# dmlc/difacto

Hardware: AMD Instinct MI355X
Metric: examples/sec (FM SGD worker step, Criteo-shape, V_dim=64) (higher is better)
Workload: dtype f32

## Files before the change

difacto_amd/csrc/dfh_localize.hip:

```cpp
#ifndef DFH_LOCALIZE_HIP_
#define DFH_LOCALIZE_HIP_
#include "dfh_internal.h"

namespace dfh {

constexpr int LOC_OVERSAMPLE = 8;
constexpr int LOC_MAX_BUCKETS = 1024;
constexpr int LOC_BIG_BUCKETS = 4096;
constexpr int LOC_AVG_BUCKET = 384;
constexpr int LOC_MIN_AVG = 48;
constexpr int LOC_MAX_AVG = 700;
constexpr int LOC_LDS_CAP = 1024;
#ifndef DFH_LOC_TILE
#define DFH_LOC_TILE 2048
#endif
#ifndef DFH_LOC_TILE_THREADS
#define DFH_LOC_TILE_THREADS 1024
#endif
constexpr int LOC_TILE = DFH_LOC_TILE;
constexpr int LOC_TILE_THREADS = DFH_LOC_TILE_THREADS;
constexpr int LOC_PER_THREAD = LOC_TILE / LOC_TILE_THREADS;
constexpr int LOC_SORT_THREADS = 256;
constexpr int LOC_EMIT_THREADS = 256;

struct LocView {
  const uint64_t* raw;
  uint32_t n;
  uint64_t max_index;
  int P;
  int bstride;
  int ntiles;
  int force_global;
  int tb;
  uint32_t nrows;
  const uint32_t* offset;
  const uint32_t* rowid;
  uint64_t* smp_key;
  uint32_t* smp_pos;
  uint32_t* smp_rank;
  uint64_t* spl_key;
  uint32_t* spl_pos;
  uint32_t* packed;
  uint32_t* run_off;
  uint32_t* btotal;
  uint32_t* bstart;
  uint64_t* bkeys;
  uint32_t* bpos;
  uint64_t* skeys;
  uint32_t* spos;
  uint64_t* first_key;
  uint64_t* last_key;
  uint32_t* nheads;
  uint32_t* lh;
  uint32_t* split_n;
};

struct SegListsOut {
  uint2* mid;
  SegEnt* mid_ent;
  uint2* hot;
  SegEnt* hot_ent;
  uint2* few;
  SegEnt* few_ent;
};

__device__ __forceinline__ uint64_t make_key(uint64_t id, uint64_t max_index) {
  const uint64_t m = (max_index == ~0ULL) ? (id == ~0ULL ? 0ULL : id) : id % max_index;
  return reverse_bytes(m);
}

constexpr int LOC_XCDS = 8;

__device__ __forceinline__ bool comp_less(uint64_t ka, uint32_t pa, uint64_t kb, uint32_t pb) {
  return ka < kb || (ka == kb && pa < pb);
}

template <bool MAX>
__device__ __forceinline__ uint32_t wave_inclusive(uint32_t x) {
#define DFH_DPP_STEP(ctrl, row_mask)                                                                      \
  {                                                                                                       \
    const uint32_t y = (uint32_t)__builtin_amdgcn_update_dpp(0, (int)x, ctrl, row_mask, 0xf, false);    \
    x = MAX ? max(x, y) : x + y;                                                                          \
  }
  DFH_DPP_STEP(0x111, 0xf)
  DFH_DPP_STEP(0x112, 0xf)
  DFH_DPP_STEP(0x114, 0xf)
  DFH_DPP_STEP(0x118, 0xf)
  DFH_DPP_STEP(0x142, 0xa)
  DFH_DPP_STEP(0x143, 0xc)
#undef DFH_DPP_STEP
  return x;
}

template <bool MAX, int NWAVES>
__device__ __forceinline__ uint32_t block_exclusive(uint32_t val, uint32_t* wtot , uint32_t* total) {
  static_assert(NWAVES <= 64, "one lane per wave");
  const int lane = (int)(threadIdx.x & 63);
  const int w = __builtin_amdgcn_readfirstlane((int)(threadIdx.x >> 6));
  const uint32_t s = wave_inclusive<MAX>(val);
  __syncthreads();
  if (lane == 63) wtot[w] = s;
  __syncthreads();
  const uint32_t x = wave_inclusive<MAX>(lane < NWAVES ? wtot[lane] : 0u);
  const uint32_t before = w ? (uint32_t)__builtin_amdgcn_readlane((int)x, w - 1) : 0u;
  if (total) *total = (uint32_t)__builtin_amdgcn_readlane((int)x, NWAVES - 1);
  const uint32_t prev = (uint32_t)__builtin_amdgcn_update_dpp(0, (int)s, 0x138, 0xf, 0xf, false);
  return MAX ? max(before, prev) : before + prev;
}
template <int NWAVES>
__device__ __forceinline__ uint32_t block_exclusive_scan(uint32_t val, uint32_t* wsum , uint32_t* total) {
  return block_exclusive<false, NWAVES>(val, wsum, total);
}
template <int NWAVES>
__device__ __forceinline__ uint32_t block_exclusive_max(uint32_t val, uint32_t* wmax , uint32_t* total) {
  return block_exclusive<true, NWAVES>(val, wmax, total);
}

__device__ __forceinline__ uint32_t ss_sample_pos(uint32_t t, uint32_t stride, uint32_t n) {
  const uint32_t j = (uint32_t)(splitmix64(t) >> 33) % stride;
  return min(t * stride + j, n - 1);
}

__global__ void __launch_bounds__(256) k_ss_sample(LocView v) {
  const uint32_t S = (uint32_t)v.P * LOC_OVERSAMPLE;
  const uint32_t stride = max(1u, v.n / S);
  for (uint32_t t = blockIdx.x * blockDim.x + threadIdx.x; t < S; t += gridDim.x * blockDim.x) {
    const uint32_t i = ss_sample_pos(t, stride, v.n);
    v.smp_key[t] = make_key(v.raw[i], v.max_index);
    v.smp_pos[t] = i << v.tb;
    v.smp_rank[t] = 0;
  }
}

__global__ void __launch_bounds__(256) k_ss_rank(LocView v) {
  __shared__ uint64_t ck[256];
  __shared__ uint32_t cp[256];
  const uint32_t S = (uint32_t)v.P * LOC_OVERSAMPLE;
  const uint32_t ntile = (S + 255) / 256;
  const uint32_t ti = blockIdx.x / ntile, tj = blockIdx.x % ntile;
  const uint32_t col = tj * 256 + threadIdx.x;
  ck[threadIdx.x] = col < S ? v.smp_key[col] : ~0ULL;
  cp[threadIdx.x] = col < S ? v.smp_pos[col] : ~0u;
  const uint32_t row = ti * 256 + threadIdx.x;
  const uint64_t mk = row < S ? v.smp_key[row] : 0;
  const uint32_t mp = row < S ? v.smp_pos[row] : 0;
  __syncthreads();
  const uint32_t lim = min(256u, S - tj * 256);
  uint32_t rank = 0;
#pragma unroll 8
  for (uint32_t j = 0; j < lim; ++j) {
    const bool less = comp_less(ck[j], cp[j], mk, mp) || (ck[j] == mk && cp[j] == mp && tj * 256 + j < row);
    rank += less ? 1u : 0u;
  }
  if (row < S && rank) atomicAdd(&v.smp_rank[row], rank);
}

__global__ void __launch_bounds__(256) k_loc_splitters(LocView v) {
  const uint32_t S = (uint32_t)v.P * LOC_OVERSAMPLE;
  for (uint32_t t = blockIdx.x * blockDim.x + threadIdx.x; t < S; t += gridDim.x * blockDim.x) {
    const uint32_t r = v.smp_rank[t];
    if (r > 0 && r % LOC_OVERSAMPLE == 0) {
      v.spl_key[r / LOC_OVERSAMPLE - 1] = v.smp_key[t];
      v.spl_pos[r / LOC_OVERSAMPLE - 1] = v.smp_pos[t];
    }
  }
}

constexpr int LOC_GATHER_ROWS = 1024;
constexpr int LOC_GATHER_SEGS = 4;
struct GatherSrc {
  int nseg;
  uint32_t seg_row0[LOC_GATHER_SEGS + 1];
  const uint32_t* src_off[LOC_GATHER_SEGS];
  const uint64_t* src_idx[LOC_GATHER_SEGS];
  const float* src_val[LOC_GATHER_SEGS];
  const uint32_t* h_rows;
  const uint32_t* h_off;
  const float* h_lab;
  const uint32_t* h_tile_row;
  uint64_t* dst_raw;
  float* dst_val;
  uint32_t* dst_off;
  float* dst_lab;
};
constexpr size_t loc_gather_smem() { return (size_t)(LOC_GATHER_ROWS + 1) * 4 + 4 + (size_t)LOC_GATHER_ROWS * 8; }
template <typename T>
__device__ __forceinline__ T loc_sel(const T (&a)[LOC_GATHER_SEGS], uint32_t sg) {
  T r = a[0];
#pragma unroll
  for (int x = 1; x < LOC_GATHER_SEGS; ++x) r = sg == (uint32_t)x ? a[x] : r;
  return r;
}

template <int MAXB>
constexpr size_t loc_count_smem() { return (size_t)MAXB * 16; }
template <int MAXB, int THREADS>
constexpr size_t loc_scatter_smem() { return (size_t)MAXB * 4 + (THREADS / 64) * 4; }
constexpr size_t loc_sort_smem() { return (size_t)LOC_LDS_CAP * 24 + 2 * (LOC_SORT_THREADS / 64) * 4; }
constexpr size_t loc_emit_smem() { return (2 * (LOC_EMIT_THREADS / 64) + 4) * 4; }

template <int MAXB, int THREADS, bool GATHER = false>
__device__ __forceinline__ void loc_count_block(const LocView& v, const uint32_t bid, const uint32_t nblk, char* smem,
                                                const GatherSrc* gp = nullptr) {
  constexpr int PER = LOC_TILE / THREADS;
  static_assert(PER * THREADS == LOC_TILE, "a tile is a whole number of elements per thread");
  uint64_t* sk = reinterpret_cast<uint64_t*>(smem);
  uint32_t* sp = reinterpret_cast<uint32_t*>(smem + (size_t)MAXB * 8);
  uint32_t* hist = sp + MAXB;
  const int P = v.P;
  for (int b = threadIdx.x; b < P; b += THREADS) {
    hist[b] = 0;
    sk[b] = b < P - 1 ? v.spl_key[b] : ~0ULL;
    sp[b] = b < P - 1 ? v.spl_pos[b] : ~0u;
  }
  const uint32_t base = bid * LOC_TILE;
  if (bid == 0 && threadIdx.x == 0 && v.split_n) *v.split_n = 0u;
  uint64_t key[PER];
  if (GATHER) {
    const GatherSrc& g = *gp;
    uint32_t* roff = reinterpret_cast<uint32_t*>(smem + loc_count_smem<MAXB>());
    uint64_t* rsrc = reinterpret_cast<uint64_t*>(roff + LOC_GATHER_ROWS + 2);
    const uint32_t row0 = g.h_tile_row[bid], row1 = g.h_tile_row[bid + 1];
    const uint32_t nr = min(row1, v.nrows - 1u) - row0 + 1u;
    for (uint32_t q = threadIdx.x; q <= nr; q += THREADS) roff[q] = g.h_off[row0 + q];
    for (uint32_t q = threadIdx.x; q < nr; q += THREADS) {
      const uint32_t r = row0 + q;
      uint32_t sg = 0;
#pragma unroll
      for (int x = 1; x < LOC_GATHER_SEGS; ++x) sg += (x < g.nseg && r >= g.seg_row0[x]) ? 1u : 0u;
      rsrc[q] = ((uint64_t)loc_sel(g.src_off, sg)[g.h_rows[r]] << 2) | sg;
    }
    __syncthreads();
#pragma unroll
    for (int e = 0; e < PER; ++e) {
      const uint32_t i = base + e * THREADS + threadIdx.x;
      key[e] = ~0ULL;
      if (i < v.n) {
        uint32_t lo = 0, hi = nr - 1u;
        while (lo < hi) {
          const uint32_t mid = (lo + hi + 1u) >> 1;
          if (roff[mid] <= i) lo = mid; else hi = mid - 1u;
        }
        const uint64_t sw = rsrc[lo];
        const uint32_t sg = (uint32_t)(sw & 3u);
        const size_t at = (size_t)(sw >> 2) + (i - roff[lo]);
        const uint64_t id = loc_sel(g.src_idx, sg)[at];
        g.dst_raw[i] = id;
        if (g.dst_val) {
          const float* sv = loc_sel(g.src_val, sg);
          g.dst_val[i] = sv ? sv[at] : 1.0f;
        }
        key[e] = make_key(id, v.max_index);
      }
    }
  } else {
#pragma unroll
    for (int e = 0; e < PER; ++e) {
      const uint32_t i = base + e * THREADS + threadIdx.x;
      key[e] = i < v.n ? make_key(v.raw[i], v.max_index) : ~0ULL;
    }
  }
  {
    uint32_t* __restrict__ rowid = const_cast<uint32_t*>(v.rowid);
    const uint32_t* __restrict__ offset = GATHER ? gp->h_off : v.offset;
    const uint32_t rpb = (v.nrows + nblk - 1) / nblk;
    const uint32_t r0 = bid * rpb, r1 = min(v.nrows, r0 + rpb);
    for (uint32_t r = r0 + threadIdx.x; r < r1; r += THREADS) {
      const uint32_t b0 = offset[r], e = offset[r + 1];
      if (GATHER) {
        gp->dst_off[r] = b0;
        gp->dst_lab[r] = gp->h_lab[r];
        if (r + 1 == v.nrows) gp->dst_off[r + 1] = e;
      }
      for (uint32_t j = b0; j < e; ++j) rowid[j] = r;
    }
  }
  __syncthreads();
  int lo[PER], hi[PER];
#pragma unroll
  for (int e = 0; e < PER; ++e) { lo[e] = 0; hi[e] = P - 1; }
  for (int step = P; step > 1; step = (step + 1) >> 1) {
#pragma unroll
    for (int e = 0; e < PER; ++e) {
      if (lo[e] < hi[e]) {
        const uint32_t i = base + e * THREADS + threadIdx.x;
        const int mid = (lo[e] + hi[e]) >> 1;
        if (comp_less(key[e], i << v.tb, sk[mid], sp[mid])) hi[e] = mid; else lo[e] = mid + 1;
      }
    }
  }
#pragma unroll
  for (int e = 0; e < PER; ++e) {
    const uint32_t i = base + e * THREADS + threadIdx.x;
    if (i < v.n) {
      const uint32_t r = atomicAdd(&hist[lo[e]], 1u);
      v.packed[i] = ((uint32_t)lo[e] << 16) | r;
    }
  }
  __syncthreads();
  for (int b = threadIdx.x; b < P; b += THREADS) {
    const uint32_t h = hist[b];
    v.run_off[bid * P + b] = h ? atomicAdd(&v.btotal[(bid & (LOC_XCDS - 1)) * MAXB + b], h) : 0u;
  }
}

template <int MAXB>
__global__ void __launch_bounds__(LOC_TILE_THREADS) k_loc_count(LocView v) {
  __shared__ __attribute__((aligned(16))) char smem[loc_count_smem<MAXB>()];
  loc_count_block<MAXB, LOC_TILE_THREADS>(v, blockIdx.x, gridDim.x, smem);
}
template <int MAXB>
__global__ void __launch_bounds__(LOC_TILE_THREADS) k_loc_count_gather(LocView v, GatherSrc g) {
  __shared__ __attribute__((aligned(16))) char smem[loc_count_smem<MAXB>() + loc_gather_smem()];
  loc_count_block<MAXB, LOC_TILE_THREADS, true>(v, blockIdx.x, gridDim.x, smem, &g);
}

constexpr int LOC_DESC_ROWS = 256;
__global__ void __launch_bounds__(LOC_DESC_ROWS) k_loc_describe(const uint32_t* __restrict__ src_off, const float* __restrict__ src_lab,
                                                                const uint32_t* __restrict__ h_rows, const uint32_t* __restrict__ h_base,
                                                                uint32_t n, uint32_t* __restrict__ dst_off, float* __restrict__ dst_lab,
                                                                int write_end) {
  __shared__ uint32_t wsum[LOC_DESC_ROWS / 64];
  const uint32_t q = blockIdx.x * LOC_DESC_ROWS + threadIdx.x;
  const bool in = q < n;
  const uint32_t r = h_rows[in ? q : n - 1u];
  const uint32_t lo = src_off[r], hi = src_off[r + 1u];
  const float lab = src_lab[r];
  const uint32_t len = in ? hi - lo : 0u;
  const uint32_t at = h_base[blockIdx.x] + block_exclusive_scan<LOC_DESC_ROWS / 64>(len, wsum, nullptr);
  if (in) {
    dst_off[q] = at;
    dst_lab[q] = lab;
    if (write_end && q + 1u == n) dst_off[n] = at + len;
  }
}


template <int MAXB, int THREADS>
__device__ __forceinline__ void loc_scatter_block(const LocView& v, const uint32_t bid, char* smem) {
  constexpr int PER = LOC_TILE / THREADS;
  constexpr int LOC_BPT = MAXB / THREADS;
  static_assert(LOC_BPT * THREADS == MAXB, "the scan of the bucket totals gives every thread the same number of buckets");
  uint32_t* off = reinterpret_cast<uint32_t*>(smem);
  uint32_t* wsum = off + MAXB;
  const int P = v.P;
  const uint32_t xcd = bid & (LOC_XCDS - 1);
  const uint32_t base = bid * LOC_TILE;
  const int b0 = threadIdx.x * LOC_BPT;
  uint32_t tt[LOC_BPT], ro[LOC_BPT];
  uint32_t sum = 0;
#pragma unroll
  for (int q = 0; q < LOC_BPT; ++q) {
    const int bb = min(b0 + q, P - 1);
    const uint32_t in = b0 + q < P ? 1u : 0u;
    tt[q] = 0;
    ro[q] = v.run_off[bid * P + bb];
#pragma unroll
    for (int x = 0; x < LOC_XCDS; ++x) {
      const uint32_t h = v.btotal[x * MAXB + bb];
      tt[q] += h;
      ro[q] += (x < (int)xcd ? 1u : 0u) * h;
    }
    tt[q] *= in;
    ro[q] *= in;
    sum += tt[q];
  }
  uint32_t total;
  uint32_t ex = block_exclusive_scan<THREADS / 64>(sum, wsum, &total);
#pragma unroll
  for (int q = 0; q < LOC_BPT; ++q) {
    if (b0 + q < P) {
      off[b0 + q] = ex + ro[q];
      if (bid == 0) v.bstart[b0 + q] = ex;
    }
    ex += tt[q];
  }
  if (bid == 0 && threadIdx.x == 0) v.bstart[P] = total;
  uint64_t raw[PER];
  uint32_t pk[PER], rw[PER];
#pragma unroll
  for (int e = 0; e < PER; ++e) {
    const uint32_t i = min(base + e * THREADS + threadIdx.x, v.n - 1);
    raw[e] = v.raw[i];
    pk[e] = v.packed[i];
    rw[e] = v.rowid[i];
  }
  __syncthreads();
#pragma unroll
  for (int e = 0; e < PER; ++e) {
    const uint32_t i = base + e * THREADS + threadIdx.x;
    if (i < v.n) {
      const uint32_t dst = off[pk[e] >> 16] + (pk[e] & 0xFFFFu);
      v.bkeys[dst] = make_key(raw[e], v.max_index);
      v.bpos[dst] = (i << v.tb) | (rw[e] & ((1u << v.tb) - 1u));
    }
  }
}

template <int MAXB>
__global__ void __launch_bounds__(LOC_TILE_THREADS) k_loc_scatter(LocView v) {
  __shared__ __attribute__((aligned(16))) char smem[loc_scatter_smem<MAXB, LOC_TILE_THREADS>()];
  loc_scatter_block<MAXB, LOC_TILE_THREADS>(v, blockIdx.x, smem);
}

__device__ __forceinline__ bool loc_sort_bucket(const LocView& v, uint32_t beg, uint32_t n, uint64_t* ak, uint32_t* ap,
                                                uint64_t* bk, uint32_t* bp, const uint64_t** sk_out, const uint32_t** sp_out) {
  const uint64_t* gk = v.bkeys + beg;
  const uint32_t* gp = v.bpos + beg;
  const bool in_lds = n <= LOC_LDS_CAP && !v.force_global;
  uint64_t* sk = bk;
  uint32_t* sp = bp;
  if (in_lds) {
    const uint32_t lane = threadIdx.x & 63;
    for (uint32_t c0 = (threadIdx.x >> 6) * 64; c0 < n; c0 += LOC_SORT_THREADS) {
      const uint32_t idx = c0 + lane;
      const bool valid = idx < n;
      const uint64_t mk = valid ? gk[idx] : ~0ULL;
      const uint32_t mp = valid ? gp[idx] : ~0u;
      const int klo = (int)(uint32_t)mk, khi = (int)(uint32_t)(mk >> 32);
      uint32_t rank = 0;
#pragma unroll 4
      for (int j = 0; j < 64; ++j) {
        const uint64_t ok = ((uint64_t)(uint32_t)__builtin_amdgcn_readlane(khi, j) << 32) | (uint32_t)__builtin_amdgcn_readlane(klo, j);
        const uint32_t op = (uint32_t)__builtin_amdgcn_readlane((int)mp, j);
        rank += comp_less(ok, op, mk, mp) ? 1u : 0u;
      }
      if (valid) {
        bk[c0 + rank] = mk;
        bp[c0 + rank] = mp;
      }
    }
    __syncthreads();
    constexpr int E = LOC_LDS_CAP / LOC_SORT_THREADS;
    constexpr int G = 2;
    static_assert(E * LOC_SORT_THREADS == LOC_LDS_CAP && E % G == 0 && LOC_SORT_THREADS % 64 == 0,
                  "a thread carries E elements of a full bucket, G at a time");
    uint64_t* dk = ak;
    uint32_t* dp = ap;
    uint32_t sh = 6;
    for (uint32_t L = 64; L < n; L <<= 1, ++sh) {
      for (int g = 0; g < E && g * LOC_SORT_THREADS < (int)n; g += G) {
        uint64_t mk[G];
        uint32_t mp[G], at[G], end[G];
#pragma unroll
        for (int e = 0; e < G; ++e) {
          const uint32_t idx = threadIdx.x + (g + e) * LOC_SORT_THREADS;
          const bool valid = idx < n;
          const uint32_t sib = ((idx >> sh) ^ 1u) << sh;
          mk[e] = valid ? sk[idx] : 0ULL;
          mp[e] = valid ? sp[idx] : 0u;
          at[e] = min(sib, n);
          end[e] = valid ? min(sib + L, n) : at[e];
        }
        for (uint32_t step = L; step; step >>= 1) {
          uint64_t ok[G];
          uint32_t op[G];
#pragma unroll
          for (int e = 0; e < G; ++e) {
            const uint32_t q = at[e] + step <= end[e] ? at[e] + step - 1u : 0u;
            ok[e] = sk[q];
            op[e] = sp[q];
          }
#pragma unroll
          for (int e = 0; e < G; ++e)
            if (at[e] + step <= end[e] && comp_less(ok[e], op[e], mk[e], mp[e])) at[e] += step;
        }
#pragma unroll
        for (int e = 0; e < G; ++e) {
          const uint32_t idx = threadIdx.x + (g + e) * LOC_SORT_THREADS;
          if (idx < n) {
            const uint32_t dst = idx + at[e] - min((idx & ~(L - 1u)) | L, n);
            dk[dst] = mk[e];
            dp[dst] = mp[e];
          }
        }
      }
      __syncthreads();
      uint64_t* tk = sk; sk = dk; dk = tk;
      uint32_t* tp = sp; sp = dp; dp = tp;
    }
    *sk_out = sk;
    *sp_out = sp;
  } else {
    uint64_t* xk = v.bkeys + beg;
    uint32_t* xp = v.bpos + beg;
    uint64_t* yk = v.skeys + beg;
    uint32_t* yp = v.spos + beg;
    const uint32_t lane = threadIdx.x & 63;
    for (uint32_t c0 = (threadIdx.x >> 6) * 64; c0 < n; c0 += LOC_SORT_THREADS) {
      const uint32_t idx = c0 + lane;
      const bool valid = idx < n;
      const uint64_t mk = valid ? xk[idx] : ~0ULL;
      const uint32_t mp = valid ? xp[idx] : ~0u;
      const uint32_t lim = min(64u, n - c0);
      uint32_t rank = 0;
      for (uint32_t j = 0; j < lim; ++j) rank += comp_less(xk[c0 + j], xp[c0 + j], mk, mp) ? 1u : 0u;
      if (valid) {
        yk[c0 + rank] = mk;
        yp[c0 + rank] = mp;
      }
    }
    __syncthreads();
    uint64_t* srck = yk; uint32_t* srcp = yp;
    uint64_t* dstk = xk; uint32_t* dstp = xp;
    for (uint32_t L = 64; L < n; L <<= 1) {
      for (uint32_t idx = threadIdx.x; idx < n; idx += blockDim.x) {
        const uint64_t mk = srck[idx];
        const uint32_t mp = srcp[idx];
        const uint32_t r = idx / L;
        const uint32_t pair_base = (r & ~1u) * L;
        const uint32_t sib = (r ^ 1u) * L;
        uint32_t lo = min(sib, n), hi = min(sib + L, n);
        const uint32_t sib_beg = lo;
        while (lo < hi) {
          const uint32_t mid = (lo + hi) >> 1;
          if (comp_less(srck[mid], srcp[mid], mk, mp)) lo = mid + 1; else hi = mid;
        }
        const uint32_t dst = pair_base + (idx - r * L) + (lo - sib_beg);
        dstk[dst] = mk;
        dstp[dst] = mp;
      }
      __syncthreads();
      uint64_t* tk = srck; srck = dstk; dstk = tk;
      uint32_t* tp = srcp; srcp = dstp; dstp = tp;
    }
    if (srck != yk) {
      for (uint32_t t = threadIdx.x; t < n; t += blockDim.x) {
        yk[t] = srck[t];
        yp[t] = srcp[t];
      }
    }
    __syncthreads();
  }
  if (!in_lds) {
    *sk_out = v.skeys + beg;
    *sp_out = v.spos + beg;
  }
  return in_lds;
}

struct BucketSummary {
  uint32_t nheads, lh;
  uint64_t first_key, last_key;
};
__device__ __forceinline__ BucketSummary loc_bucket_summary(const uint64_t* sk, uint32_t n, uint32_t (*red)[LOC_SORT_THREADS / 64]) {
  uint32_t cnt = 0, last = 0;
  for (uint32_t t = 1 + threadIdx.x; t < n; t += blockDim.x) {
    if (sk[t] != sk[t - 1]) {
      ++cnt;
      last = t;
    }
  }
  cnt = (uint32_t)__builtin_amdgcn_readlane((int)wave_inclusive<false>(cnt), 63);
  last = (uint32_t)__builtin_amdgcn_readlane((int)wave_inclusive<true>(last), 63);
  if ((threadIdx.x & 63) == 0) {
    red[0][threadIdx.x >> 6] = cnt;
    red[1][threadIdx.x >> 6] = last;
  }
  __syncthreads();
  BucketSummary r;
  r.nheads = 1;
  r.lh = 0;
  r.first_key = 0;
  r.last_key = 0;
  if (threadIdx.x == 0) {
    for (int w = 0; w < LOC_SORT_THREADS / 64; ++w) {
      r.nheads += red[0][w];
      r.lh = max(r.lh, red[1][w]);
    }
    r.first_key = sk[0];
    r.last_key = sk[n - 1];
  }
  return r;
}

__device__ __forceinline__ void loc_sort_block(const LocView& v, const uint32_t bid, const uint32_t nblk, char* smem) {
  uint64_t* ak = reinterpret_cast<uint64_t*>(smem);
  uint64_t* bk = ak + LOC_LDS_CAP;
  uint32_t* ap = reinterpret_cast<uint32_t*>(bk + LOC_LDS_CAP);
  uint32_t* bp = ap + LOC_LDS_CAP;
  uint32_t (*red)[LOC_SORT_THREADS / 64] = reinterpret_cast<uint32_t (*)[LOC_SORT_THREADS / 64]>(bp + LOC_LDS_CAP);
  for (uint32_t b = bid; b < (uint32_t)v.P; b += nblk) {
    __syncthreads();
    const uint32_t beg = v.bstart[b], end = v.bstart[b + 1];
    const uint32_t n = end - beg;
    if (threadIdx.x < LOC_XCDS) v.btotal[threadIdx.x * v.bstride + b] = 0;
    if (n == 0) {
      if (threadIdx.x == 0) {
        v.nheads[b] = 0;
        v.lh[b] = 0;
        v.first_key[b] = 0;
        v.last_key[b] = 0;
      }
      continue;
    }
    const uint64_t* sk;
    const uint32_t* sp;
    if (loc_sort_bucket(v, beg, n, ak, ap, bk, bp, &sk, &sp)) {
      for (uint32_t t = threadIdx.x; t < n; t += LOC_SORT_THREADS) {
        v.skeys[beg + t] = sk[t];
        v.spos[beg + t] = sp[t];
      }
    }
    const BucketSummary sm = loc_bucket_summary(sk, n, red);
    if (threadIdx.x == 0) {
      v.nheads[b] = sm.nheads;
      v.lh[b] = sm.lh;
      v.first_key[b] = sm.first_key;
      v.last_key[b] = sm.last_key;
    }
  }
}
__global__ void __launch_bounds__(LOC_SORT_THREADS) k_loc_sort(LocView v) {
  extern __shared__ __attribute__((aligned(16))) char smem[];
  loc_sort_block(v, blockIdx.x, gridDim.x, smem);
}

template <int NW, bool PROBE>
__device__ __forceinline__ void loc_emit_bucket(const LocView& v, uint32_t b, uint32_t beg, uint32_t n, const uint64_t* sk,
                                                const uint32_t* sp, uint32_t cont, uint32_t ubase, uint32_t carry1,
                                                const float* __restrict__ value,
                                                uint64_t* __restrict__ feaids, uint32_t* __restrict__ col_ptr,
                                                uint32_t* __restrict__ index, uint32_t* __restrict__ s_row,
                                                float* __restrict__ s_val, uint32_t* __restrict__ d_U, const SegListsOut& sl,
                                                uint32_t* wsum, uint32_t* wmax, uint32_t* n_mid, uint32_t* n_hot,
                                                uint32_t* n_few, const TableView& tab, uint32_t* __restrict__ urow) {
  const uint32_t P = (uint32_t)v.P;
  const uint32_t moff = beg / (BWD_SMALL + 1) + 2 * b, hoff = beg / (BWD_MID + 1) + 2 * b, foff = beg / 2 + 2 * b;
  uint32_t run_heads = 0, run_max1 = carry1;
  for (uint32_t base = 0; base < n; base += blockDim.x) {
    const uint32_t t = base + threadIdx.x;
    const uint32_t i = beg + t;
    const bool valid = t < n;
    uint64_t key = 0;
    uint32_t tag = 0;
    bool head = false;
    if (valid) {
      key = sk[t];
      tag = sp[t];
      head = t == 0 ? !cont : key != sk[t - 1];
    }
    const uint32_t pos = tag >> v.tb;
    uint32_t nh, mx;
    const uint32_t ex = block_exclusive_scan<NW>(head ? 1u : 0u, wsum, &nh);
    const uint32_t pm = block_exclusive_max<NW>(head ? i + 1 : 0u, wmax, &mx);
    if (valid) {
      const uint32_t incl = run_heads + ex + (head ? 1u : 0u);
      const uint32_t uid = ubase + incl - 1;
      const uint32_t prev1 = max(run_max1, pm);
      if (head) {
        feaids[uid] = key;
        col_ptr[uid] = i;
        if (PROBE) urow[uid] = find_or_insert(tab, key);
        if (prev1) {
          const uint32_t len = i - (prev1 - 1);
          const SegEnt e = make_uint4(uid - 1, prev1 - 1, i, 0u);
          if (len > BWD_MID) sl.hot_ent[hoff + atomicAdd(n_hot, 1u)] = e;
          else if (len > BWD_SMALL) sl.mid_ent[moff + atomicAdd(n_mid, 1u)] = e;
          else if (len > 1) sl.few_ent[foff + atomicAdd(n_few, 1u)] = e;
        }
      }
      index[pos] = uid;
      uint32_t row = tag & ((1u << v.tb) - 1u);
      {
        const uint32_t step = 1u << v.tb;
        uint32_t lo = 0, hi = v.nrows > row ? (v.nrows - 1u - row) >> v.tb : 0u;
        while (lo < hi) {
          const uint32_t mid = (lo + hi + 1u) >> 1;
          if (v.offset[row + mid * step] <= pos) lo = mid; else hi = mid - 1u;
        }
        row += lo * step;
      }
      s_row[i] = row;
      if (value) s_val[i] = value[pos];
      if (i == v.n - 1) {
        *d_U = uid + 1;
        col_ptr[uid + 1] = v.n;
        const uint32_t lbeg = head ? i : prev1 - 1, len = v.n - lbeg;
        const SegEnt e = make_uint4(uid, lbeg, v.n, 0u);
        if (len > BWD_MID) sl.hot_ent[hoff + atomicAdd(n_hot, 1u)] = e;
        else if (len > BWD_SMALL) sl.mid_ent[moff + atomicAdd(n_mid, 1u)] = e;
        else if (len > 1) sl.few_ent[foff + atomicAdd(n_few, 1u)] = e;
      }
    }
    run_heads += nh;
    run_max1 = max(run_max1, mx);
  }
  if (P > 1) {
    const uint64_t N = v.n;
    const uint64_t m0 = max((uint64_t)beg * P / N + ((uint64_t)beg * P % N ? 1u : 0u), (uint64_t)1);
    const uint64_t e1 = (uint64_t)(beg + n) * P;
    const uint64_t m1 = min(e1 / N + (e1 % N ? 1u : 0u), (uint64_t)P);
    for (uint64_t m = m0 + threadIdx.x; m < m1; m += blockDim.x) {
      const uint32_t i = (uint32_t)(m * N / P);
      if ((i * (uint64_t)P + N - 1) / N == m) {
        v.spl_key[m - 1] = sk[i - beg];
        v.spl_pos[m - 1] = sp[i - beg];
      }
    }
  }
  __syncthreads();
  if (threadIdx.x == 0) {
    sl.mid[b] = make_uint2(*n_mid, moff);
    sl.hot[b] = make_uint2(*n_hot, hoff);
    sl.few[b] = make_uint2(*n_few, foff);
  }
}

struct EmitOut {
  const float* value;
  uint64_t* feaids;
  uint32_t* col_ptr;
  uint32_t* index;
  uint32_t* s_row;
  float* s_val;
  uint32_t* d_U;
  SegListsOut sl;
};

template <bool PROBE>
__device__ __forceinline__ void loc_emit_block(const LocView& v, const EmitOut& o, const TableView& tab, uint32_t* __restrict__ urow,
                                               const uint32_t bid, const uint32_t nblk, char* smem) {
  constexpr int NW = LOC_EMIT_THREADS / 64;
  uint32_t* wsum = reinterpret_cast<uint32_t*>(smem);
  uint32_t* wmax = wsum + NW;
  uint32_t& sh_cont = wmax[NW];
  uint32_t& n_mid = wmax[NW + 1];
  uint32_t& n_hot = wmax[NW + 2];
  uint32_t& n_few = wmax[NW + 3];
  const SegListsOut& sl = o.sl;
  const uint32_t P = (uint32_t)v.P;
  for (uint32_t b = bid; b < P; b += nblk) {
    __syncthreads();
    const uint32_t beg = v.bstart[b], end = v.bstart[b + 1];
    const uint32_t n = end - beg;
    if (threadIdx.x == 0) {
      n_mid = 0;
      n_hot = 0;
      n_few = 0;
      if (n == 0) {
        sl.mid[b] = make_uint2(0u, 0u);
        sl.hot[b] = make_uint2(0u, 0u);
        sl.few[b] = make_uint2(0u, 0u);
      }
    }
    if (n == 0) continue;
    uint32_t part = 0, carry1 = 0;
    for (uint32_t q0 = threadIdx.x; q0 <= b; q0 += LOC_EMIT_THREADS) {
      const uint32_t bq = v.bstart[q0], nq = v.bstart[q0 + 1] - bq;
      if (nq == 0) continue;
      int p = (int)q0 - 1;
      while (p >= 0 && v.bstart[p + 1] == v.bstart[p]) --p;
      const uint32_t c = (p >= 0 && v.first_key[q0] == v.last_key[p]) ? 1u : 0u;
      if (q0 == b) {
        sh_cont = c;
      } else {
        part += v.nheads[q0] - c;
        const uint32_t l = v.lh[q0];
        if (l > 0) carry1 = max(carry1, bq + l + 1);
        else if (!c) carry1 = max(carry1, bq + 1);
      }
    }
    uint32_t ubase, carry_all;
    block_exclusive_scan<NW>(part, wsum, &ubase);
    block_exclusive_max<NW>(carry1, wmax, &carry_all);
    __syncthreads();
    loc_emit_bucket<NW, PROBE>(v, b, beg, n, v.skeys + beg, v.spos + beg, sh_cont, ubase, carry_all, o.value, o.feaids, o.col_ptr,
                               o.index, o.s_row, o.s_val, o.d_U, sl, wsum, wmax, &n_mid, &n_hot, &n_few, tab, urow);
  }
}

template <bool PROBE>
__global__ void __launch_bounds__(LOC_EMIT_THREADS) k_loc_emit(LocView v, EmitOut o, TableView tab, uint32_t* __restrict__ urow) {
  __shared__ __attribute__((aligned(16))) char smem[loc_emit_smem()];
  loc_emit_block<PROBE>(v, o, tab, urow, blockIdx.x, gridDim.x, smem);
}

}
#endif
```

Baseline: 85.77 million.

## Sort 64-element runs with an in-register bitonic network and fuse writeback into summary

Measured after the change: 88.81 million, median of 6. 1.04x the previous value.

```diff
diff --git a/difacto_amd/csrc/dfh_localize.hip b/difacto_amd/csrc/dfh_localize.hip
--- a/difacto_amd/csrc/dfh_localize.hip
+++ b/difacto_amd/csrc/dfh_localize.hip
@@ -403,152 +403,208 @@
   loc_scatter_block<MAXB, LOC_TILE_THREADS>(v, blockIdx.x, smem);
 }
 
-__device__ __forceinline__ bool loc_sort_bucket(const LocView& v, uint32_t beg, uint32_t n, uint64_t* ak, uint32_t* ap,
-                                                uint64_t* bk, uint32_t* bp, const uint64_t** sk_out, const uint32_t** sp_out) {
+template <int J>
+__device__ __forceinline__ uint32_t loc_net_partner(uint32_t x) {
+  static_assert(J == 1 || J == 2 || J == 4 || J == 8, "DPP reaches the partners inside a row of 16 lanes");
+  if constexpr (J == 1) return (uint32_t)__builtin_amdgcn_mov_dpp((int)x, 0xB1, 0xf, 0xf, false);
+  if constexpr (J == 2) return (uint32_t)__builtin_amdgcn_mov_dpp((int)x, 0x4E, 0xf, 0xf, false);
+  if constexpr (J == 4) {
+    const int y = __builtin_amdgcn_mov_dpp((int)x, 0x141, 0xf, 0xf, false);
+    return (uint32_t)__builtin_amdgcn_mov_dpp(y, 0x1B, 0xf, 0xf, false);
+  }
+  return (uint32_t)__builtin_amdgcn_mov_dpp((int)x, 0x128, 0xf, 0xf, false);
+}
+constexpr uint64_t loc_net_keeps_max(int K, int J) {
+  uint64_t m = 0;
+  for (int i = 0; i < 64; ++i) m |= (uint64_t)(((i & J) != 0) != ((i & K) != 0)) << i;
+  return m;
+}
+template <int K, int J>
+__device__ __forceinline__ void loc_net_stage(uint32_t& klo, uint32_t& khi, uint32_t& tag) {
+  uint32_t mlo, mhi;
+  asm volatile("s_mov_b32 %0, %2\n\ts_mov_b32 %1, %3"
+               : "=s"(mlo), "=s"(mhi)
+               : "i"((int32_t)(uint32_t)loc_net_keeps_max(K, J)), "i"((int32_t)(uint32_t)(loc_net_keeps_max(K, J) >> 32)));
+  const uint64_t mask = ((uint64_t)mhi << 32) | mlo;
+  const bool keeps_max = __builtin_amdgcn_inverse_ballot_w64(mask);
+  if constexpr (J >= 16) {
+    uint32_t alo, ahi, at, blo, bhi, bt;
+#define DFH_NET_SWAP(a, b, x)                                                                                       \
+    {                                                                                                                 \
+      const auto r = J == 16 ? __builtin_amdgcn_permlane16_swap(x, x, false, false) : __builtin_amdgcn_permlane32_swap(x, x, false, false); \
+      a = r[0];                                                                                                       \
+      b = r[1];                                                                                                       \
+    }
+    DFH_NET_SWAP(alo, blo, klo)
+    DFH_NET_SWAP(ahi, bhi, khi)
+    DFH_NET_SWAP(at, bt, tag)
+#undef DFH_NET_SWAP
+    const bool out_of_order = comp_less(((uint64_t)bhi << 32) | blo, bt, ((uint64_t)ahi << 32) | alo, at);
+    const bool take_b = out_of_order != keeps_max;
+    klo = take_b ? blo : alo;
+    khi = take_b ? bhi : ahi;
+    tag = take_b ? bt : at;
+  } else {
+    const uint32_t olo = loc_net_partner<J>(klo), ohi = loc_net_partner<J>(khi), ot = loc_net_partner<J>(tag);
+    const bool partner_less = comp_less(((uint64_t)ohi << 32) | olo, ot, ((uint64_t)khi << 32) | klo, tag);
+    const bool take = partner_less != keeps_max;
+    klo = take ? olo : klo;
+    khi = take ? ohi : khi;
+    tag = take ? ot : tag;
+  }
+}
+template <int K, int J>
+__device__ __forceinline__ void loc_net_merge(uint32_t& klo, uint32_t& khi, uint32_t& tag) {
+  loc_net_stage<K, J>(klo, khi, tag);
+  if constexpr (J > 1) loc_net_merge<K, J / 2>(klo, khi, tag);
+}
+template <int K = 2>
+__device__ __forceinline__ void loc_net_sort64(uint32_t& klo, uint32_t& khi, uint32_t& tag) {
+  loc_net_merge<K, K / 2>(klo, khi, tag);
+  if constexpr (K < 64) loc_net_sort64<K * 2>(klo, khi, tag);
+}
+
+__device__ __forceinline__ bool loc_sort_bucket_lds(const LocView& v, uint32_t beg, uint32_t n, uint64_t* ak, uint32_t* ap,
+                                                    uint64_t* bk, uint32_t* bp) {
   const uint64_t* gk = v.bkeys + beg;
   const uint32_t* gp = v.bpos + beg;
-  const bool in_lds = n <= LOC_LDS_CAP && !v.force_global;
   uint64_t* sk = bk;
   uint32_t* sp = bp;
-  if (in_lds) {
-    const uint32_t lane = threadIdx.x & 63;
-    for (uint32_t c0 = (threadIdx.x >> 6) * 64; c0 < n; c0 += LOC_SORT_THREADS) {
-      const uint32_t idx = c0 + lane;
-      const bool valid = idx < n;
-      const uint64_t mk = valid ? gk[idx] : ~0ULL;
-      const uint32_t mp = valid ? gp[idx] : ~0u;
-      const int klo = (int)(uint32_t)mk, khi = (int)(uint32_t)(mk >> 32);
-      uint32_t rank = 0;
-#pragma unroll 4
-      for (int j = 0; j < 64; ++j) {
-        const uint64_t ok = ((uint64_t)(uint32_t)__builtin_amdgcn_readlane(khi, j) << 32) | (uint32_t)__builtin_amdgcn_readlane(klo, j);
-        const uint32_t op = (uint32_t)__builtin_amdgcn_readlane((int)mp, j);
-        rank += comp_less(ok, op, mk, mp) ? 1u : 0u;
-      }
-      if (valid) {
-        bk[c0 + rank] = mk;
-        bp[c0 + rank] = mp;
+  const uint32_t lane = threadIdx.x & 63;
+  for (uint32_t c0 = (threadIdx.x >> 6) * 64; c0 < n; c0 += LOC_SORT_THREADS) {
+    const uint32_t idx = c0 + lane;
+    const bool valid = idx < n;
+    const uint64_t mk = valid ? gk[idx] : ~0ULL;
+    uint32_t klo = (uint32_t)mk, khi = (uint32_t)(mk >> 32);
+    uint32_t mp = valid ? gp[idx] : ~0u;
+    loc_net_sort64(klo, khi, mp);
+    if (valid) {
+      bk[idx] = ((uint64_t)khi << 32) | klo;
+      bp[idx] = mp;
+    }
+  }
+  __syncthreads();
+  constexpr int E = LOC_LDS_CAP / LOC_SORT_THREADS;
+  constexpr int G = 2;
+  static_assert(E * LOC_SORT_THREADS == LOC_LDS_CAP && E % G == 0 && LOC_SORT_THREADS % 64 == 0,
+                "a thread carries E elements of a full bucket, G at a time");
+  uint64_t* dk = ak;
+  uint32_t* dp = ap;
+  uint32_t sh = 6;
+  for (uint32_t L = 64; L < n; L <<= 1, ++sh) {
+    for (int g = 0; g < E && g * LOC_SORT_THREADS < (int)n; g += G) {
+      uint64_t mk[G];
+      uint32_t mp[G], at[G], end[G];
+#pragma unroll
+      for (int e = 0; e < G; ++e) {
+        const uint32_t idx = threadIdx.x + (g + e) * LOC_SORT_THREADS;
+        const bool valid = idx < n;
+        const uint32_t sib = ((idx >> sh) ^ 1u) << sh;
+        mk[e] = valid ? sk[idx] : 0ULL;
+        mp[e] = valid ? sp[idx] : 0u;
+        at[e] = min(sib, n);
+        end[e] = valid ? min(sib + L, n) : at[e];
+      }
+      for (uint32_t step = L; step; step >>= 1) {
+        uint64_t ok[G];
+        uint32_t op[G];
+#pragma unroll
+        for (int e = 0; e < G; ++e) {
+          const uint32_t q = at[e] + step <= end[e] ? at[e] + step - 1u : 0u;
+          ok[e] = sk[q];
+          op[e] = sp[q];
+        }
+#pragma unroll
+        for (int e = 0; e < G; ++e)
+          if (at[e] + step <= end[e] && comp_less(ok[e], op[e], mk[e], mp[e])) at[e] += step;
+      }
+#pragma unroll
+      for (int e = 0; e < G; ++e) {
+        const uint32_t idx = threadIdx.x + (g + e) * LOC_SORT_THREADS;
+        if (idx < n) {
+          const uint32_t dst = idx + at[e] - min((idx & ~(L - 1u)) | L, n);
+          dk[dst] = mk[e];
+          dp[dst] = mp[e];
+        }
       }
     }
     __syncthreads();
-    constexpr int E = LOC_LDS_CAP / LOC_SORT_THREADS;
-    constexpr int G = 2;
-    static_assert(E * LOC_SORT_THREADS == LOC_LDS_CAP && E % G == 0 && LOC_SORT_THREADS % 64 == 0,
-                  "a thread carries E elements of a full bucket, G at a time");
-    uint64_t* dk = ak;
-    uint32_t* dp = ap;
-    uint32_t sh = 6;
-    for (uint32_t L = 64; L < n; L <<= 1, ++sh) {
-      for (int g = 0; g < E && g * LOC_SORT_THREADS < (int)n; g += G) {
-        uint64_t mk[G];
-        uint32_t mp[G], at[G], end[G];
-#pragma unroll
-        for (int e = 0; e < G; ++e) {
-          const uint32_t idx = threadIdx.x + (g + e) * LOC_SORT_THREADS;
-          const bool valid = idx < n;
-          const uint32_t sib = ((idx >> sh) ^ 1u) << sh;
-          mk[e] = valid ? sk[idx] : 0ULL;
-          mp[e] = valid ? sp[idx] : 0u;
-          at[e] = min(sib, n);
-          end[e] = valid ? min(sib + L, n) : at[e];
-        }
-        for (uint32_t step = L; step; step >>= 1) {
-          uint64_t ok[G];
-          uint32_t op[G];
-#pragma unroll
-          for (int e = 0; e < G; ++e) {
-            const uint32_t q = at[e] + step <= end[e] ? at[e] + step - 1u : 0u;
-            ok[e] = sk[q];
-            op[e] = sp[q];
-          }
-#pragma unroll
-          for (int e = 0; e < G; ++e)
-            if (at[e] + step <= end[e] && comp_less(ok[e], op[e], mk[e], mp[e])) at[e] += step;
-        }
-#pragma unroll
-        for (int e = 0; e < G; ++e) {
-          const uint32_t idx = threadIdx.x + (g + e) * LOC_SORT_THREADS;
-          if (idx < n) {
-            const uint32_t dst = idx + at[e] - min((idx & ~(L - 1u)) | L, n);
-            dk[dst] = mk[e];
-            dp[dst] = mp[e];
-          }
-        }
-      }
-      __syncthreads();
-      uint64_t* tk = sk; sk = dk; dk = tk;
-      uint32_t* tp = sp; sp = dp; dp = tp;
-    }
-    *sk_out = sk;
-    *sp_out = sp;
-  } else {
-    uint64_t* xk = v.bkeys + beg;
-    uint32_t* xp = v.bpos + beg;
-    uint64_t* yk = v.skeys + beg;
-    uint32_t* yp = v.spos + beg;
-    const uint32_t lane = threadIdx.x & 63;
-    for (uint32_t c0 = (threadIdx.x >> 6) * 64; c0 < n; c0 += LOC_SORT_THREADS) {
-      const uint32_t idx = c0 + lane;
-      const bool valid = idx < n;
-      const uint64_t mk = valid ? xk[idx] : ~0ULL;
-      const uint32_t mp = valid ? xp[idx] : ~0u;
-      const uint32_t lim = min(64u, n - c0);
-      uint32_t rank = 0;
-      for (uint32_t j = 0; j < lim; ++j) rank += comp_less(xk[c0 + j], xp[c0 + j], mk, mp) ? 1u : 0u;
-      if (valid) {
-        yk[c0 + rank] = mk;
-        yp[c0 + rank] = mp;
-      }
+    uint64_t* tk = sk; sk = dk; dk = tk;
+    uint32_t* tp = sp; sp = dp; dp = tp;
+  }
+  return sk == ak;
+}
+__device__ __forceinline__ void loc_sort_bucket_global(const LocView& v, uint32_t beg, uint32_t n) {
+  uint64_t* xk = v.bkeys + beg;
+  uint32_t* xp = v.bpos + beg;
+  uint64_t* yk = v.skeys + beg;
+  uint32_t* yp = v.spos + beg;
+  const uint32_t lane = threadIdx.x & 63;
+  for (uint32_t c0 = (threadIdx.x >> 6) * 64; c0 < n; c0 += LOC_SORT_THREADS) {
+    const uint32_t idx = c0 + lane;
+    const bool valid = idx < n;
+    const uint64_t mk = valid ? xk[idx] : ~0ULL;
+    const uint32_t mp = valid ? xp[idx] : ~0u;
+    const uint32_t lim = min(64u, n - c0);
+    uint32_t rank = 0;
+    for (uint32_t j = 0; j < lim; ++j) rank += comp_less(xk[c0 + j], xp[c0 + j], mk, mp) ? 1u : 0u;
+    if (valid) {
+      yk[c0 + rank] = mk;
+      yp[c0 + rank] = mp;
+    }
+  }
+  __syncthreads();
+  uint64_t* srck = yk; uint32_t* srcp = yp;
+  uint64_t* dstk = xk; uint32_t* dstp = xp;
+  for (uint32_t L = 64; L < n; L <<= 1) {
+    for (uint32_t idx = threadIdx.x; idx < n; idx += blockDim.x) {
+      const uint64_t mk = srck[idx];
+      const uint32_t mp = srcp[idx];
+      const uint32_t r = idx / L;
+      const uint32_t pair_base = (r & ~1u) * L;
+      const uint32_t sib = (r ^ 1u) * L;
+      uint32_t lo = min(sib, n), hi = min(sib + L, n);
+      const uint32_t sib_beg = lo;
+      while (lo < hi) {
+        const uint32_t mid = (lo + hi) >> 1;
+        if (comp_less(srck[mid], srcp[mid], mk, mp)) lo = mid + 1; else hi = mid;
+      }
+      const uint32_t dst = pair_base + (idx - r * L) + (lo - sib_beg);
+      dstk[dst] = mk;
+      dstp[dst] = mp;
     }
     __syncthreads();
-    uint64_t* srck = yk; uint32_t* srcp = yp;
-    uint64_t* dstk = xk; uint32_t* dstp = xp;
-    for (uint32_t L = 64; L < n; L <<= 1) {
-      for (uint32_t idx = threadIdx.x; idx < n; idx += blockDim.x) {
-        const uint64_t mk = srck[idx];
-        const uint32_t mp = srcp[idx];
-        const uint32_t r = idx / L;
-        const uint32_t pair_base = (r & ~1u) * L;
-        const uint32_t sib = (r ^ 1u) * L;
-        uint32_t lo = min(sib, n), hi = min(sib + L, n);
-        const uint32_t sib_beg = lo;
-        while (lo < hi) {
-          const uint32_t mid = (lo + hi) >> 1;
-          if (comp_less(srck[mid], srcp[mid], mk, mp)) lo = mid + 1; else hi = mid;
-        }
-        const uint32_t dst = pair_base + (idx - r * L) + (lo - sib_beg);
-        dstk[dst] = mk;
-        dstp[dst] = mp;
-      }
-      __syncthreads();
-      uint64_t* tk = srck; srck = dstk; dstk = tk;
-      uint32_t* tp = srcp; srcp = dstp; dstp = tp;
-    }
-    if (srck != yk) {
-      for (uint32_t t = threadIdx.x; t < n; t += blockDim.x) {
-        yk[t] = srck[t];
-        yp[t] = srcp[t];
-      }
-    }
-    __syncthreads();
-  }
-  if (!in_lds) {
-    *sk_out = v.skeys + beg;
-    *sp_out = v.spos + beg;
-  }
-  return in_lds;
+    uint64_t* tk = srck; srck = dstk; dstk = tk;
+    uint32_t* tp = srcp; srcp = dstp; dstp = tp;
+  }
+  if (srck != yk) {
+    for (uint32_t t = threadIdx.x; t < n; t += blockDim.x) {
+      yk[t] = srck[t];
+      yp[t] = srcp[t];
+    }
+  }
+  __syncthreads();
 }
 
 struct BucketSummary {
   uint32_t nheads, lh;
   uint64_t first_key, last_key;
 };
-__device__ __forceinline__ BucketSummary loc_bucket_summary(const uint64_t* sk, uint32_t n, uint32_t (*red)[LOC_SORT_THREADS / 64]) {
+template <bool WRITE>
+__device__ __forceinline__ BucketSummary loc_bucket_summary(const uint64_t* sk, const uint32_t* sp, uint32_t n, uint64_t* ok,
+                                                            uint32_t* op, uint32_t (*red)[LOC_SORT_THREADS / 64]) {
   uint32_t cnt = 0, last = 0;
-  for (uint32_t t = 1 + threadIdx.x; t < n; t += blockDim.x) {
-    if (sk[t] != sk[t - 1]) {
+  uint32_t t0 = threadIdx.x;
+  asm volatile("" : "+v"(t0));
+  for (uint32_t t = t0; t < n; t += LOC_SORT_THREADS) {
+    const uint64_t k = sk[t];
+    if (WRITE) {
+      ok[t] = k;
+      op[t] = sp[t];
+    }
+    if (t + 1 < n && sk[t + 1] != k) {
       ++cnt;
-      last = t;
+      last = t + 1;
     }
   }
   cnt = (uint32_t)__builtin_amdgcn_readlane((int)wave_inclusive<false>(cnt), 63);
@@ -594,15 +650,14 @@
       }
       continue;
     }
-    const uint64_t* sk;
-    const uint32_t* sp;
-    if (loc_sort_bucket(v, beg, n, ak, ap, bk, bp, &sk, &sp)) {
-      for (uint32_t t = threadIdx.x; t < n; t += LOC_SORT_THREADS) {
-        v.skeys[beg + t] = sk[t];
-        v.spos[beg + t] = sp[t];
-      }
-    }
-    const BucketSummary sm = loc_bucket_summary(sk, n, red);
+    BucketSummary sm;
+    if (n <= LOC_LDS_CAP && !v.force_global) {
+      const bool in_a = loc_sort_bucket_lds(v, beg, n, ak, ap, bk, bp);
+      sm = loc_bucket_summary<true>(in_a ? ak : bk, in_a ? ap : bp, n, v.skeys + beg, v.spos + beg, red);
+    } else {
+      loc_sort_bucket_global(v, beg, n);
+      sm = loc_bucket_summary<false>(v.skeys + beg, v.spos + beg, n, nullptr, nullptr, red);
+    }
     if (threadIdx.x == 0) {
       v.nheads[b] = sm.nheads;
       v.lh[b] = sm.lh;
```
